# deemoe404/rmcv

Measured on AMD Instinct MI355X. Metric: frames/sec (1280x1024 BGR) armour detect, higher is better.
Workload: dtype u8

## Files before the change

### rmcv_amd/csrc/k_contours.hip

```cpp
#include "contours_device.h"

namespace rmcv {

#define KC_KERNEL k_contours_w8
#define KC_THREADS 512
#include "k_contours_kernel.inc"
#undef KC_KERNEL
#undef KC_THREADS

static_assert(sizeof(ContoursLds) >= (CT_THREADS_MAX / 64) * sizeof(WaveLds), "the fit rows reuse the contour tables");

bool sparse_lean_applies(const Geom& g, const Bufs& b)
{
    return g.sparse_lean && !g.dense_defer && g.contour_tier == 0 && b.mid && g.h <= CT_MAXH && g.ww <= 32;
}

static hipError_t launch_contours_x(const Geom& g, const Bufs& b, const Limits& lim, const SparseTail& X, int waves, hipStream_t s)
{
    SparseSched Q;
    Q.order = b.frame_order;
    const int grid = g.n_frames;
    static const int force_literal = getenv("RMCV_CONTOURS_LITERAL") ? atoi(getenv("RMCV_CONTOURS_LITERAL")) : 0;
    static bool attr_set[MAX_DEVICES] = {};
    if (!attr_set[g.device]) {
        hipError_t e = hipFuncSetAttribute(reinterpret_cast<const void*>(k_contours_w8), hipFuncAttributeMaxDynamicSharedMemorySize,
                                           (int)lds_bytes(CT_MAXH));
        if (e != hipSuccess) return e;
        attr_set[g.device] = true;
    }
    const int force = force_literal ? force_literal : g.contour_tier;
    if (waves == 4 && X.fused && !X.C.enabled && sparse_lean_applies(g, b) && force == 0) return launch_contours_lean(g, b, lim, X, 2, Q, grid, s);
    if (waves == 4) {
        const bool defer = g.dense_defer && (force & 3) == 0 && b.mid;
        if (g.dense_defer == 3 && !defer) return hipSuccess;
        hipError_t e = g.dense_defer == 3 ? hipSuccess : launch_contours_w4(g, b, lim, X, force | (defer ? 4 : 0), Q, grid, s);
        if (e != hipSuccess || !defer || g.dense_defer == 2) return e;
        const SparseSched& Q2 = Q;
        static const bool second_w4 = getenv("RMCV_DEFER_W4") && atoi(getenv("RMCV_DEFER_W4"));
        if (second_w4) return launch_contours_w4(g, b, lim, X, 2 | 8, Q2, grid, s);
        return launch(k_contours_w8, dim3(grid), dim3(512), lds_bytes(g.h), s, b.bits, b.rowmask, g.h, b.lab, b.neg, g.w,
                       g.h, g.ww, g.prow, g.plane_pitch, b.points, b.cont_start, b.cont_len, b.n_contours, b.n_points, b.status,
                       lim.max_contours, lim.max_points, 2 | 8, b.elig, b.n_elig, b.slot_kind, X, b.visit_xy, b.mid, b.mid_stride,
                       b.mid_slot_cap, Q2, lds_rows_cap(g.h));
    }
    return launch(k_contours_w8, dim3(grid), dim3(512), lds_bytes(g.h), s, b.bits, b.rowmask, g.h, b.lab, b.neg, g.w,
                       g.h, g.ww, g.prow, g.plane_pitch, b.points, b.cont_start, b.cont_len, b.n_contours, b.n_points, b.status,
                       lim.max_contours, lim.max_points, force, b.elig, b.n_elig, b.slot_kind, X, b.visit_xy, b.mid, b.mid_stride,
                       b.mid_slot_cap, Q, lds_rows_cap(g.h));
}

hipError_t launch_contours(const Geom& g, const Bufs& b, const Limits& lim, hipStream_t s)
{
    SparseTail X;
    memset(&X, 0, sizeof(X));
    return launch_contours_x(g, b, lim, X, 8, s);
}

hipError_t launch_sparse(const Geom& g, const Bufs& b, const Limits& lim, const rmcv_params& p, bool pairs, bool identity, int waves, hipStream_t s)
{
    SparseTail X;
    memset(&X, 0, sizeof(X));
    X.fused = 1;
    X.G = {p.tilt_max, p.ratio_lo, p.ratio_hi, p.area_lo, p.area_hi, g.overloads};
    X.slot_ell = b.slot_ell;
    FitTail& T = X.T;
    T.blobs = b.blobs;
    T.blob_src = b.blob_src;
    T.ellipses = b.ellipses;
    T.neg_idx = b.neg_idx;
    T.n_blobs = b.n_blobs;
    T.n_neg = b.n_neg;
    T.status = b.status;
    T.armours = b.armours;
    T.n_armours = b.n_armours;
    T.max_blobs = lim.max_blobs;
    T.max_armours = lim.max_armours;
    T.enemy = p.camp;
    T.do_pairs = pairs ? 1 : 0;
    T.angle_diff_max = p.angle_diff_max;
    T.shear_max = p.shear_max;
    T.length_ratio_max = p.length_ratio_max;
    T.ov = g.overloads;
    if (identity && pairs) X.C = classify_args(g, b);
    return launch_contours_x(g, b, lim, X, waves, s);
}

__device__ __forceinline__ void export_lists(const ExportArgs& a, int gtid, int nthreads)
{
    if (gtid < 12 && a.hdr_src[gtid]) a.hdr_dst[gtid] = *a.hdr_src[gtid];
    for (int k = 0; k < a.n_sec; k++) {
        const ExportSec& e = a.sec[k];
        int n = e.count ? e.count[0] + e.count_add : e.max_elems;
        n = n < 0 ? 0 : (n > e.max_elems ? e.max_elems : n);
        const int ndw = n * (e.elem_bytes >> 2);
        const uint32_t* src = static_cast<const uint32_t*>(e.src);
        uint32_t* dst = static_cast<uint32_t*>(e.dst);
        for (int i = gtid; i < ndw; i += nthreads) dst[i] = src[i];
    }
}

__global__ void k_export(ExportArgs a)
{
    export_lists(a, blockIdx.x * blockDim.x + threadIdx.x, gridDim.x * blockDim.x);
}

hipError_t launch_export(const ExportArgs& a, hipStream_t s)
{
    return launch(k_export, dim3(8), dim3(256), 0, s, a);
}

__global__ void k_pack_contours(const rmcv_point* __restrict__ points, const int32_t* __restrict__ cont_start,
                                const int32_t* __restrict__ cont_len, const int32_t* __restrict__ n_contours, int max_contours,
                                int max_points, rmcv_point* __restrict__ pts_out, int32_t* __restrict__ offs_out,
                                int32_t* __restrict__ hdr_out, const int32_t* __restrict__ status, ExportArgs ex)
// ... 95 lines not shown
```

### rmcv_amd/csrc/rmcv_host.hip

```cpp
#include <math.h>
#include <sched.h>
#include <time.h>
#include <stdio.h>
#include <stdlib.h>
#include <string.h>

#include <algorithm>
#include <vector>

#include "rmcv_internal.h"

using namespace rmcv;

struct rmcv_ctx {
    int device = 0;
    Limits lim{};
    Geom geom{};
    Bufs bufs{};
    hipStream_t stream = nullptr;
    hipEvent_t ev[6] = {};
    uint8_t* own_frames = nullptr;
    size_t own_frames_bytes = 0;
    rmcv_point* pack_pts = nullptr;
    int32_t* pack_offs = nullptr;
// ... 266 lines not shown
    if (e == hipSuccess) {
        hipDeviceProp_t prop;
        c->geom.device = device;
        c->geom.pixel_halo_nt = getenv("RMCV_K1_HALO_NT") ? atoi(getenv("RMCV_K1_HALO_NT")) : 0;
        c->geom.pixel_rowquad = getenv("RMCV_K1_LINEAR") && atoi(getenv("RMCV_K1_LINEAR")) == 0;
        if (getenv("RMCV_IMAGE_EXPORT")) c->image_export = atoi(getenv("RMCV_IMAGE_EXPORT"));
        if (getenv("RMCV_FRAME_UPLOAD")) c->frame_upload = atoi(getenv("RMCV_FRAME_UPLOAD"));
        c->geom.pixel_ws = 1;
        c->geom.dense_defer = getenv("RMCV_DENSE_DEFER") ? atoi(getenv("RMCV_DENSE_DEFER")) : 0;
        c->geom.n_cu = (device < MAX_DEVICES && hipGetDeviceProperties(&prop, device) == hipSuccess) ? prop.multiProcessorCount : 0;
        if (device >= MAX_DEVICES) e = hipErrorInvalidDevice;
    }
    const size_t F = (size_t)d.max_frames;
    const size_t plane = (size_t)(d.max_height + 2) * ((d.max_width + 63) / 64 + 2);
    Bufs& b = c->bufs;
    if (e == hipSuccess) e = dalloc(c, &b.binary, F * d.max_width * d.max_height);
    if (e == hipSuccess) e = dalloc(c, &b.bits, F * plane);
    if (e == hipSuccess) e = dalloc(c, &b.rowmask, F * d.max_height);
    if (e == hipSuccess) e = dalloc(c, &b.strip_ctr, 9 * CTR_STRIDE);
    if (e == hipSuccess) e = dalloc(c, &b.lab, F * plane);
    if (e == hipSuccess) e = dalloc(c, &b.neg, F * plane);
    if (e == hipSuccess) e = dalloc(c, &b.points, F * d.max_points);
    if (e == hipSuccess) e = dalloc(c, &c->pack_pts, F * d.max_points);
    if (e == hipSuccess) e = dalloc(c, &c->pack_offs, F * (d.max_contours + 1));
    if (e == hipSuccess) e = dalloc(c, &b.cont_start, F * d.max_contours);
    if (e == hipSuccess) e = dalloc(c, &b.cont_len, F * d.max_contours);
    if (e == hipSuccess) e = dalloc(c, &b.n_contours, F);
    if (e == hipSuccess) e = dalloc(c, &b.n_points, F);
    if (e == hipSuccess) e = dalloc(c, &b.visit_xy, F * VISIT_CAP);
    {
        const int64_t words = (int64_t)((d.max_width + 63) / 64) * d.max_height;
        b.mid_slot_cap = (int)std::min<int64_t>(words, 65535);
        b.mid_stride = (int64_t)((mid_bytes(b.mid_slot_cap) + 255) & ~(size_t)255);
        b.mid = nullptr;
    }
    if (e == hipSuccess) e = dalloc(c, &b.blobs, F * d.max_blobs);
    if (e == hipSuccess) e = dalloc(c, &b.blob_src, F * d.max_blobs);
    if (e == hipSuccess) e = dalloc(c, &b.ellipses, F * d.max_blobs);
    if (e == hipSuccess) e = dalloc(c, &b.neg_idx, F * d.max_contours);
    if (e == hipSuccess) e = dalloc(c, &b.elig, F * d.max_contours);
    if (e == hipSuccess) e = dalloc(c, &b.n_elig, F);
    if (e == hipSuccess) e = dalloc(c, &b.slot_kind, F * d.max_contours);
    if (e == hipSuccess) e = dalloc(c, &b.slot_ell, F * d.max_contours);
    if (e == hipSuccess) e = dalloc(c, &b.n_blobs, F);
    if (e == hipSuccess) e = dalloc(c, &b.n_neg, F);
    if (e == hipSuccess) e = dalloc(c, &b.armours, F * d.max_armours);
    if (e == hipSuccess) e = dalloc(c, &b.n_armours, F);
    if (e == hipSuccess) e = dalloc(c, &b.status, F);
    if (e == hipSuccess) e = dalloc(c, &b.frame_order, F);
    if (e == hipSuccess) e = dalloc(c, &c->order_scratch, 2 * F);
    if (e == hipSuccess) {
        hipMemset(b.strip_ctr, 0, 9 * CTR_STRIDE * sizeof(int));
        hipMemset(b.n_contours, 0, F * 4);
        hipMemset(b.n_points, 0, F * 4);
        hipMemset(b.n_blobs, 0, F * 4);
        hipMemset(b.n_neg, 0, F * 4);
        hipMemset(b.n_armours, 0, F * 4);
        e = hipMemset(b.status, 0, F * 4);
    }
    if (e != hipSuccess) {
        fprintf(stderr, "rmcv_ctx_create: %s\n", hipGetErrorString(e));
        rmcv_ctx_destroy(c);
        return e == hipErrorOutOfMemory ? RMCV_ERR_NOMEM : RMCV_ERR_HIP;
    }
    *out = c;
    return RMCV_OK;
}

}

namespace rmcv {
void ctx_external_order(rmcv_ctx* c, hipEvent_t done)
{
    c->external_order = true;
    c->ext_done = done;
}
const Limits& ctx_limits(const rmcv_ctx* c) { return c->lim; }
void ctx_pixel_shape(rmcv_ctx* c, int shape) { c->geom.pixel_ws = shape ? 1 : 0; }
uint64_t ctx_blocking_calls(const rmcv_ctx* c) { return c->blocking_calls; }
int ctx_wait_timeout_ms(const rmcv_ctx* c) { return c->wait_timeout_ms; }
bool pixel_ws_full(const rmcv_ctx* c, int lower_bound) { return binary_ws_full(c->geom, c->bufs, lower_bound); }
void ctx_defer_phase(rmcv_ctx* c, int phase) { c->geom.dense_defer = phase; }
void ctx_sparse_lean(rmcv_ctx* c, int on) { c->geom.sparse_lean = on ? 1 : 0; }
int ctx_input_format(const rmcv_ctx* c) { return c->input_format; }
int ctx_compact(rmcv_ctx* c, void* d_armours_out, int cap, void* d_frame_offs, void* d_status_or, hipStream_t s, void* hd_record, int host_head)
{
    HIPCHK(c, launch_compact_armours(c->geom, c->bufs, c->lim, (rmcv_armour*)d_armours_out, cap, (int32_t*)d_frame_offs, s, (int32_t*)d_status_or, (uint8_t*)hd_record, host_head), "k_compact_armours");
    return RMCV_OK;
}
}

static void resident_none(rmcv_ctx* c)
{
    c->res_nc = c->res_nb = -1;
    c->ahead_lb = c->ahead_ar = false;
}

static int ensure_own_frames(rmcv_ctx* c, size_t need)
{
    if (need <= c->own_frames_bytes) return RMCV_OK;
    if (c->own_frames) hipFree(c->own_frames);
    c->own_frames = nullptr;
    c->own_frames_bytes = 0;
    size_t cap = (size_t)((3 * c->lim.max_width + 15) & ~15) * c->lim.max_height * c->lim.max_frames;
    if (cap < need) cap = need;
    HIPCHK(c, hipMalloc((void**)&c->own_frames, cap), "hipMalloc frames");
    c->own_frames_bytes = cap;
    return RMCV_OK;
}

static int ensure_staging(rmcv_ctx* c)
{
    if (c->h_hdr) return RMCV_OK;
    const Limits& L = c->lim;
    hipError_t e = hipHostMalloc((void**)&c->h_hdr, 16 * sizeof(int32_t), hipHostMallocDefault);
    if (e == hipSuccess) e = hipHostMalloc((void**)&c->h_pts, (size_t)L.max_points * sizeof(rmcv_point), hipHostMallocDefault);
    if (e == hipSuccess) e = hipHostMalloc((void**)&c->h_offs, (size_t)(L.max_contours + 1) * 4, hipHostMallocDefault);
    if (e == hipSuccess) e = hipHostMalloc((void**)&c->h_blobs, (size_t)L.max_blobs * sizeof(rmcv_lightblob), hipHostMallocDefault);
    if (e == hipSuccess) e = hipHostMalloc((void**)&c->h_blob_src, (size_t)L.max_blobs * 4, hipHostMallocDefault);
    if (e == hipSuccess) e = hipHostMalloc((void**)&c->h_neg, (size_t)L.max_contours * 4, hipHostMallocDefault);
    if (e == hipSuccess) e = hipHostMalloc((void**)&c->h_armours, (size_t)L.max_armours * sizeof(rmcv_armour), hipHostMallocDefault);
    if (e == hipSuccess) e = dalloc(c, &c->d_hdr, 16);
    if (e != hipSuccess) return fail(c, RMCV_ERR_NOMEM, "pinned staging", e);
    memset(c->h_hdr, 0, 16 * sizeof(int32_t));
    if (hipHostGetDevicePointer((void**)&c->hd_hdr, c->h_hdr, 0) != hipSuccess || hipHostGetDevicePointer((void**)&c->hd_pts, c->h_pts, 0) != hipSuccess ||
        hipHostGetDevicePointer((void**)&c->hd_offs, c->h_offs, 0) != hipSuccess || hipHostGetDevicePointer((void**)&c->hd_blobs, c->h_blobs, 0) != hipSuccess ||
        hipHostGetDevicePointer((void**)&c->hd_blob_src, c->h_blob_src, 0) != hipSuccess || hipHostGetDevicePointer((void**)&c->hd_neg, c->h_neg, 0) != hipSuccess ||
        hipHostGetDevicePointer((void**)&c->hd_armours, c->h_armours, 0) != hipSuccess) {
        (void)hipGetLastError();
        c->hd_hdr = nullptr;
    }
    return RMCV_OK;
}

static int ensure_mid(rmcv_ctx* c, int n_frames)
{
    if (n_frames <= c->mid_frames || c->mid_failed) return RMCV_OK;
    const bool no_mid = getenv("RMCV_NO_MID") && atoi(getenv("RMCV_NO_MID"));
    c->blocking_calls++;
    if (c->bufs.mid) {
        const int rcs = rmcv_batch_sync(c);
        if (rcs) return rcs;
        uint8_t* raw = c->bufs.mid - GUARD;
        for (size_t i = 0; i < c->allocs.size(); i++)
            if (c->allocs[i] == raw) { c->allocs.erase(c->allocs.begin() + i); break; }
        for (size_t i = 0; i < c->guarded.size(); i++)
            if (c->guarded[i].base == raw) { c->guarded.erase(c->guarded.begin() + i); break; }
        (void)hipFree(raw);
        c->bufs.mid = nullptr;
        c->mid_frames = 0;
    }
    const int want = n_frames > 1 ? c->lim.max_frames : 1;
    uint8_t* m = nullptr;
    const hipError_t e = no_mid ? hipErrorOutOfMemory : dalloc_named(c, &m, (size_t)want * (size_t)c->bufs.mid_stride, "b.mid");
    if (e != hipSuccess) {
        (void)hipGetLastError();
        c->mid_failed = true;
        return RMCV_OK;
    }
    c->bufs.mid = m;
    c->mid_frames = want;
    return RMCV_OK;
}

namespace rmcv {
static constexpr int ORDER_LDS = 2048;
// ... 1408 lines not shown
```

### rmcv_amd/csrc/rmcv_internal.h

```cpp
#pragma once
#include <hip/hip_runtime.h>
#include <stdint.h>

#include <tuple>
#include <utility>

#include "../../include/rmcv_abi.h"

namespace rmcv {

struct Geom {
    int device;
    int n_cu;
    int pixel_halo_nt;
    int pixel_rowquad;
    int pixel_ws;
    int dense_defer;
    int overloads;
    int sparse_lean;
    int contour_tier;
    int input_format;
    int n_frames;
    int w, h;
    int stride;
    int64_t frame_pitch;
    int ww;
    int prow;
    int64_t plane_pitch;
};

static constexpr int CTR_STRIDE = 32;
#ifndef RMCV_SR
#define RMCV_SR 32
#endif
static constexpr int STRIP_ROWS = RMCV_SR;
static constexpr int VISIT_CAP = 4096;
static constexpr int NN_MID = 1 << 17;
static constexpr int CAND_MID = 1 << 15;
inline size_t mid_bytes(int slot_cap)
{
    return (size_t)slot_cap * (6 * 8 + 2 * 4) + (size_t)NN_MID * (2 * 8 + 2 * 4) + (size_t)CAND_MID * 4 * 4;
}

struct Limits {
    int max_frames, max_width, max_height, max_contours, max_points, max_blobs, max_armours;
};

struct Bufs {
    const uint8_t* frames;
    uint8_t* binary;
    uint64_t* bits;
    int* strip_ctr;
    uint32_t* rowmask;
    uint64_t* lab;
    uint64_t* neg;
    rmcv_point* points;
    int32_t* cont_start;
    int32_t* cont_len;
    int32_t* n_contours;
    int32_t* n_points;
    uint32_t* visit_xy;
    uint8_t* mid;
    int64_t mid_stride;
    int mid_slot_cap;
    rmcv_lightblob* blobs;
    int32_t* blob_src;
    rmcv_rrect* ellipses;
    int32_t* elig;
    int32_t* n_elig;
    int32_t* slot_kind;
    rmcv_rrect* slot_ell;
    int32_t* neg_idx;
    int32_t* n_blobs;
    int32_t* n_neg;
    rmcv_armour* armours;
    int32_t* n_armours;
    int32_t* status;
    int32_t* frame_order;
    float* svm_w;
    double* svm_rho;
    int32_t* svm_labels;
    int svm_classes;
    int32_t* identity;
    uint8_t* icons;
    rmcv_pnp_config* pnp_cfg;
    double* base2gripper;
    double* poses;
};

#define RMCV_FRAME_DEFERRED_ (1 << 30)

struct SparseSched {
    const int32_t* order;
};

static constexpr int MAX_DEVICES = 64;

template <typename... P, size_t... I>
inline hipError_t launch_tuple(void (*kernel)(P...), dim3 grid, dim3 block, size_t lds, hipStream_t s, std::tuple<P...>& vals,
                               std::index_sequence<I...>)
{
    void* ptrs[] = {static_cast<void*>(const_cast<typename std::remove_const<P>::type*>(&std::get<I>(vals)))...};
    return hipLaunchKernel(reinterpret_cast<const void*>(kernel), grid, block, ptrs, lds, s);
}
template <typename... P, typename... A>
inline hipError_t launch(void (*kernel)(P...), dim3 grid, dim3 block, size_t lds, hipStream_t s, A&&... a)
{
    static_assert(sizeof...(P) == sizeof...(A), "argument count differs from the kernel's parameter list");
    std::tuple<P...> vals{static_cast<P>(a)...};
    return launch_tuple(kernel, grid, block, lds, s, vals, std::index_sequence_for<P...>{});
}

int64_t pixel_ws_launches();
hipError_t launch_match(const Geom& g, const Bufs& b, const Limits& lim, const rmcv_params& p, const rmcv_legacy_params& lp,
                        int mode, bool with_frames, bool pairs, hipStream_t s);
hipError_t launch_sparse(const Geom& g, const Bufs& b, const Limits& lim, const rmcv_params& p, bool pairs, bool identity, int waves, hipStream_t s);
hipError_t launch_pnp(const Geom& g, const Bufs& b, const Limits& lim, hipStream_t s);
hipError_t launch_binary(const Geom& g, const Bufs& b, int camp, int lower_bound, int morph, bool image, int groups, hipStream_t s);
bool binary_ws_full(const Geom& g, const Bufs& b, int lower_bound);
hipError_t launch_binary_bayer(const Geom& g, const Bufs& b, int camp, int lower_bound, int morph, bool image, hipStream_t s);
hipError_t launch_demosaic(const uint8_t* d_raw, int stride, int w, int h, int pattern, uint8_t* d_out, int out_stride, hipStream_t s);
bool sparse_lean_applies(const Geom& g, const Bufs& b);
hipError_t launch_contours(const Geom& g, const Bufs& b, const Limits& lim, hipStream_t s);
hipError_t launch_blobs(const Geom& g, const Bufs& b, const Limits& lim, const rmcv_params& p, hipStream_t s);
hipError_t launch_armours(const Geom& g, const Bufs& b, const Limits& lim, const rmcv_params& p, hipStream_t s);
hipError_t launch_blobs_armours(const Geom& g, const Bufs& b, const Limits& lim, const rmcv_params& p, hipStream_t s);
hipError_t launch_compact_armours(const Geom& g, const Bufs& b, const Limits& lim, rmcv_armour* d_out, int cap,
                                  int32_t* d_frame_offs, hipStream_t s, int32_t* d_status_or = nullptr, uint8_t* hd_record = nullptr, int host_head = 0);
hipError_t launch_status_clear(const Geom& g, const Bufs& b, int mask, hipStream_t s);
hipError_t launch_classify(const Geom& g, const Bufs& b, const Limits& lim, hipStream_t s);
hipError_t launch_pack_bits(const Geom& g, const Bufs& b, hipStream_t s);
struct ExportSec {
    const void* src;
    void* dst;
    const int32_t* count;
    int count_add, elem_bytes, max_elems;
};
struct ExportArgs {
    ExportSec sec[8];
    int n_sec;
    const int32_t* hdr_src[12];
    int32_t* hdr_dst;
};
hipError_t launch_export(const ExportArgs& a, hipStream_t s);
hipError_t launch_pack_contours(const Geom& g, const Bufs& b, const Limits& lim, rmcv_point* d_pts_out, int32_t* d_offs_out,
                                int32_t* d_hdr , hipStream_t s, const ExportArgs* ex = nullptr);
hipError_t launch_gather3(const int32_t* a, const int32_t* b, const int32_t* c, int32_t* d_out, hipStream_t s);

void ctx_external_order(rmcv_ctx* c, hipEvent_t done);
int ctx_compact(rmcv_ctx* c, void* d_armours_out, int cap, void* d_frame_offs, void* d_status_or, hipStream_t s, void* hd_record = nullptr, int host_head = 0);
const Limits& ctx_limits(const rmcv_ctx* c);
void ctx_pixel_shape(rmcv_ctx* c, int shape);
int ctx_bind_frames(rmcv_ctx* c, const void* d_frames, int n_frames, int w, int h, int stride, int64_t frame_pitch, hipStream_t s);
int ctx_prepare_ring(rmcv_ctx* c);
uint64_t ctx_blocking_calls(const rmcv_ctx* c);
int ctx_wait_timeout_ms(const rmcv_ctx* c);
bool pixel_ws_full(const rmcv_ctx* c, int lower_bound);
int wait_stream_deadline(hipStream_t s, int timeout_ms, hipError_t* err);
int wait_event_deadline(hipEvent_t ev, int timeout_ms, hipError_t* err);
hipError_t launch_delay(unsigned long long ns, hipStream_t s);
int ctx_check_stages(rmcv_ctx* c, const rmcv_params* p, int stages);
void ctx_defer_phase(rmcv_ctx* c, int phase);
void ctx_sparse_lean(rmcv_ctx* c, int on);
int ctx_input_format(const rmcv_ctx* c);

}
```

### rmcv_amd/csrc/rmcv_pipeline.hip

```cpp
#include <stdio.h>
#include <stdlib.h>
#include <string.h>
#include <time.h>

#include <new>
#include <vector>

#include "rmcv_internal.h"

using namespace rmcv;


struct rmcv_pipeline {
    int device = 0;
    rmcv_pipeline_config cfg{};
    Limits lim{};
    int64_t head_bytes = 0, record_bytes = 0;
    std::vector<rmcv_ctx*> ring;
    std::vector<hipStream_t> pix, sp, dn;
    std::vector<hipEvent_t> ev_bin, ev_done, ev_host, ev_sp;
    std::vector<void*> ev_hook;
    std::vector<uint8_t*> d_rec, h_rec, hd_rec;
    std::vector<uint64_t> slot_ticket;
    std::vector<int> slot_frames;
    std::vector<hipStream_t> slot_stream;
    uint64_t next_ticket = 0, collected = 0;
    int hot = 0;
    bool calm = false;
    uint64_t hot_seq = 0, hot_batches = 0;
    std::vector<int> ctx_last;
    std::vector<int> slot_ctx;
    std::vector<hipEvent_t> ev_free;
    struct Pending {
        bool valid = false;
        uint64_t t = 0;
        size_t k = 0;
        rmcv_ctx* c = nullptr;
        rmcv_params p{};
        rmcv_legacy_params lp{};
        bool has_lp = false, used = false, heavy = false;
        int sparse = 0, n_frames = 0;
        hipStream_t B = nullptr;
    } pend;
    uint64_t latency_batches = 0;
    bool lazy_back = true;
    bool chain_cold = true, was_cold = false;
    int chain_cold_us = 60;
    bool early_free = true;
    bool heavy = false;
    int heavy_pixel_groups = 0;
    uint64_t heavy_batches = 0;
    std::vector<char> slot_lean;
    bool split_now = false;
    uint64_t split_batches = 0;
    rmcv_pipeline_hook hook = nullptr;
    void* hook_user = nullptr;
    rmcv_comm* comm = nullptr;
    int root = 0, n_ranks = 0, rank = 0;
    std::vector<uint8_t*> d_recv;
    hipEvent_t ev_gather = nullptr;
    bool gather_pending = false;
    uint64_t blocking_base = 0, own_blocking = 0, held_back = 0;
    std::vector<hipEvent_t> ev_chg;
    int wait_timeout_ms = 5000;
    const char* last_what = "nothing";
    int hot_cfg = 0;
    int64_t hot_plane_bytes = 0;
    bool ws_always = false;
    bool hot_identity = false;
    double max_submit_us = 0;
    char err[256] = {0};
};

static int finish_back(rmcv_pipeline* pl, bool latency);
static int hot_for(const rmcv_pipeline* pl, int n_frames, int w, int h);

static int pfail(rmcv_pipeline* pl, int code, const char* what, hipError_t e = hipSuccess)
{
    if (pl) {
        if (e != hipSuccess) snprintf(pl->err, sizeof(pl->err), "%s: %s", what, hipGetErrorString(e));
        else snprintf(pl->err, sizeof(pl->err), "%s", what);
    }
    if (e != hipSuccess) (void)hipGetLastError();
    return code;
}
#define PCHK(pl, call, what)                                               \
    do {                                                                   \
        (pl)->last_what = what;                                            \
        hipError_t e__ = (call);                                           \
        if (e__ != hipSuccess) return pfail((pl), RMCV_ERR_HIP, what, e__); \
    } while (0)
static int cfail(rmcv_pipeline* pl, rmcv_ctx* c, int rc)
{
    snprintf(pl->err, sizeof(pl->err), "%s", rmcv_last_error(c));
    return rc;
}

static int pwait_event(rmcv_pipeline* pl, hipEvent_t ev, const char* what)
{
    hipError_t e = hipSuccess;
    const int rcw = wait_event_deadline(ev, pl->wait_timeout_ms, &e);
    if (rcw < 0) return pfail(pl, RMCV_ERR_HIP, what, e);
    if (rcw > 0) {
        snprintf(pl->err, sizeof(pl->err), "%s: not finished after %d ms (rmcv_pipeline_set_wait_timeout); enqueued last: %s", what, pl->wait_timeout_ms, pl->last_what);
        return RMCV_ERR_TIMEOUT;
    }
    return RMCV_OK;
}
static int pwait_stream(rmcv_pipeline* pl, hipStream_t st, const char* what)
{
    hipError_t e = hipSuccess;
    const int rcw = wait_stream_deadline(st, pl->wait_timeout_ms, &e);
    if (rcw < 0) return pfail(pl, RMCV_ERR_HIP, what, e);
    if (rcw > 0) {
        snprintf(pl->err, sizeof(pl->err), "%s: not finished after %d ms (rmcv_pipeline_set_wait_timeout); enqueued last: %s", what, pl->wait_timeout_ms, pl->last_what);
        return RMCV_ERR_TIMEOUT;
    }
    return RMCV_OK;
}
static uint64_t ring_blocking(const rmcv_pipeline* pl)
{
    uint64_t n = 0;
    for (auto c : pl->ring) n += ctx_blocking_calls(c);
    return n;
}

extern "C" {

void rmcv_default_pipeline_config(rmcv_pipeline_config* c)
{
    if (!c) return;
    memset(c, 0, sizeof(*c));
    c->depth = 8;
    c->pixel_streams = 2;
    c->sparse_streams = 4;
    c->armour_cap = 0;
    c->sparse_waves = 4;
    c->pixel_groups = 2;
    c->host_results = 1;
    c->dense_streams = 4;
    c->hot_contexts = 0;
}

void rmcv_pipeline_destroy(rmcv_pipeline* pl)
{
    if (!pl) return;
    hipSetDevice(pl->device);
    if (!pl->ring.empty()) (void)finish_back(pl, true);
    {
        bool stuck = false;
        for (auto s : pl->pix) if (s) stuck |= pwait_stream(pl, s, "destroy") == RMCV_ERR_TIMEOUT;
// ... 56 lines not shown
    for (int k = 0; k < d.depth && rc == RMCV_OK; k++) {
        rmcv_ctx* c = nullptr;
        rc = rmcv_ctx_create(device, limits, &c);
        if (rc == RMCV_OK) {
            pl->ring.push_back(c);
            rc = rmcv_ctx_set_option(c, RMCV_OPT_SPARSE_WAVES, d.sparse_waves);
            if (rc == RMCV_OK) rc = rmcv_ctx_set_option(c, RMCV_OPT_PIXEL_GROUPS, d.pixel_groups);
            if (rc == RMCV_OK) rc = ctx_prepare_ring(c);
        }
    }
    if (rc != RMCV_OK) {
        rmcv_pipeline_destroy(pl);
        return rc;
    }
    pl->lim = ctx_limits(pl->ring[0]);
    if (pl->cfg.armour_cap <= 0) pl->cfg.armour_cap = 8 * pl->lim.max_frames;
    pl->head_bytes = (((int64_t)pl->lim.max_frames + 3) * 4 + 15) / 16 * 16;
    pl->record_bytes = pl->head_bytes + (int64_t)pl->cfg.armour_cap * (int64_t)sizeof(rmcv_armour);
    hipError_t e = hipSetDevice(device);
    int lo = 0, hi = 0;
    if (e == hipSuccess) e = hipDeviceGetStreamPriorityRange(&lo, &hi);
    for (int i = 0; i < d.pixel_streams && e == hipSuccess; i++) {
        hipStream_t s = nullptr;
        e = hipStreamCreateWithPriority(&s, hipStreamNonBlocking, 0);
        pl->pix.push_back(s);
    }
    for (int i = 0; i < d.sparse_streams && e == hipSuccess; i++) {
        hipStream_t s = nullptr;
        e = hipStreamCreateWithPriority(&s, hipStreamNonBlocking, hi);
        pl->sp.push_back(s);
    }
    const unsigned dev_flags = hipEventDisableTiming;
    for (int i = 0; i < d.dense_streams && e == hipSuccess; i++) {
        hipStream_t s = nullptr;
        e = hipStreamCreateWithPriority(&s, hipStreamNonBlocking, 0);
        pl->dn.push_back(s);
    }
    for (int k = 0; k < d.depth && e == hipSuccess; k++) {
        hipEvent_t a = nullptr, b = nullptr, h = nullptr, sp_ = nullptr;
        if (e == hipSuccess) e = hipEventCreateWithFlags(&sp_, hipEventDisableTiming);
        pl->ev_sp.push_back(sp_);
        hipEvent_t fr_ = nullptr, chg_ = nullptr;
        if (e == hipSuccess) e = hipEventCreateWithFlags(&fr_, hipEventDisableTiming);
        pl->ev_free.push_back(fr_);
        if (e == hipSuccess) e = hipEventCreateWithFlags(&chg_, hipEventDisableTiming);
        pl->ev_chg.push_back(chg_);
        uint8_t *dr = nullptr, *hr = nullptr;
        e = hipEventCreateWithFlags(&a, dev_flags);
        if (e == hipSuccess) e = hipEventCreateWithFlags(&b, dev_flags);
        if (e == hipSuccess) e = hipEventCreateWithFlags(&h, hipEventDisableTiming);
        if (e == hipSuccess) e = hipMalloc((void**)&dr, (size_t)pl->record_bytes);
        if (e == hipSuccess) e = hipMemset(dr, 0, (size_t)pl->record_bytes);
        uint8_t* hdr = nullptr;
        if (e == hipSuccess && d.host_results == 1) {
            e = hipHostMalloc((void**)&hr, (size_t)pl->record_bytes, hipHostMallocMapped);
            if (e == hipSuccess) memset(hr, 0, (size_t)pl->record_bytes);
            if (e == hipSuccess) e = hipHostGetDevicePointer((void**)&hdr, hr, 0);
        }
        pl->hd_rec.push_back(hdr);
        pl->ev_bin.push_back(a);
        pl->ev_done.push_back(b);
        pl->ev_host.push_back(h);
        pl->d_rec.push_back(dr);
        pl->h_rec.push_back(hr);
        pl->ev_hook.push_back(nullptr);
        pl->slot_ticket.push_back(0);
        pl->slot_frames.push_back(0);
        pl->slot_stream.push_back(nullptr);
        if (e == hipSuccess) ctx_external_order(pl->ring[(size_t)k], b);
    }
    if (e == hipSuccess) e = hipEventCreateWithFlags(&pl->ev_gather, hipEventDisableTiming);
    pl->ctx_last.assign((size_t)d.depth, -1);
    pl->slot_lean.assign((size_t)d.depth, 0);
    pl->slot_ctx.assign((size_t)d.depth, 0);
    pl->hot = hot_for(pl, pl->lim.max_frames, pl->lim.max_width, pl->lim.max_height);
    pl->wait_timeout_ms = ctx_wait_timeout_ms(pl->ring[0]);
#ifdef RMCV_DEV_KNOBS
    pl->lazy_back = !(getenv("RMCV_LAZY_BACK") && atoi(getenv("RMCV_LAZY_BACK")) == 0);
    pl->chain_cold = !(getenv("RMCV_CHAIN_COLD") && atoi(getenv("RMCV_CHAIN_COLD")) == 0);
    if (getenv("RMCV_CHAIN_COLD")) pl->chain_cold_us = atoi(getenv("RMCV_CHAIN_COLD")) > 1 ? atoi(getenv("RMCV_CHAIN_COLD")) : 0;
    pl->early_free = !(getenv("RMCV_EARLY_FREE") && atoi(getenv("RMCV_EARLY_FREE")) == 0);
    if (getenv("RMCV_HOT_IDENTITY")) pl->hot_identity = atoi(getenv("RMCV_HOT_IDENTITY")) != 0;
    if (getenv("RMCV_WS_ALWAYS")) pl->ws_always = atoi(getenv("RMCV_WS_ALWAYS")) != 0;
    if (getenv("RMCV_HEAVY_PG")) pl->heavy_pixel_groups = atoi(getenv("RMCV_HEAVY_PG")) > 0 ? atoi(getenv("RMCV_HEAVY_PG")) : 0;
    if (getenv("RMCV_HEAVY_OFF") && atoi(getenv("RMCV_HEAVY_OFF"))) pl->heavy_pixel_groups = -1;
#endif
    pl->blocking_base = ring_blocking(pl);
    if (e != hipSuccess) {
        fprintf(stderr, "rmcv_pipeline_create: %s\n", hipGetErrorString(e));
        (void)hipGetLastError();
        rmcv_pipeline_destroy(pl);
        return e == hipErrorOutOfMemory ? RMCV_ERR_NOMEM : RMCV_ERR_HIP;
    }
    *out = pl;
    return RMCV_OK;
}

int rmcv_hw_queues_hint(void)
{
    setenv("GPU_MAX_HW_QUEUES", "12", 0);
    const char* q = getenv("GPU_MAX_HW_QUEUES");
    return q ? atoi(q) : 0;
}

const char* rmcv_pipeline_last_error(const rmcv_pipeline* pl) { return pl ? pl->err : "null pipeline"; }

int rmcv_pipeline_get_info(const rmcv_pipeline* pl, rmcv_pipeline_info* o)
{
    if (!pl || !o) return RMCV_ERR_BAD_ARG;
    memset(o, 0, sizeof(*o));
    o->depth = pl->cfg.depth;
    o->pixel_streams = pl->cfg.pixel_streams;
    o->sparse_streams = pl->cfg.sparse_streams;
    o->armour_cap = pl->cfg.armour_cap;
    o->sparse_waves = pl->cfg.sparse_waves;
    o->pixel_groups = pl->cfg.pixel_groups;
    o->host_results = pl->cfg.host_results;
    o->dense_streams = pl->cfg.dense_streams;
    o->max_frames = pl->lim.max_frames;
    const char* q = getenv("GPU_MAX_HW_QUEUES");
    o->hw_queues_env = q ? atoi(q) : 0;
    o->hw_queues_wanted = 1 + pl->cfg.pixel_streams + pl->cfg.sparse_streams + pl->cfg.dense_streams + (pl->comm ? 1 : 0);
    o->record_bytes = pl->record_bytes;
    o->armours_offset = pl->head_bytes;
    o->submitted = pl->next_ticket;
    o->collected = pl->collected;
    o->dense_split = pl->split_batches;
    o->hot_batches = pl->hot_batches;
    o->hot_contexts = pl->hot;
    o->latency_batches = pl->latency_batches;
    o->host_blocking_calls = pl->own_blocking;
    o->max_submit_us = pl->max_submit_us;
    o->wait_timeout_ms = pl->wait_timeout_ms;
    o->held_back = pl->held_back;
    o->heavy_batches = pl->heavy_batches;
    return RMCV_OK;
}

rmcv_ctx* rmcv_pipeline_context(rmcv_pipeline* pl, int slot)
{
    if (!pl || slot < 0 || slot >= pl->cfg.depth) return nullptr;
    return pl->ring[(size_t)slot];
}

int rmcv_pipeline_set_hot_contexts(rmcv_pipeline* pl, int n)
{
    if (!pl) return RMCV_ERR_BAD_ARG;
    if (n <= 0) { pl->hot = 0; pl->hot_cfg = -1; return RMCV_OK; }
    if (n < 3 || n >= pl->cfg.depth) return pfail(pl, RMCV_ERR_BAD_ARG, "hot_contexts: 3 .. depth - 1, or 0 / -1 for off");
    if (pl->cfg.host_results != 1 || pl->cfg.sparse_waves != 4) return pfail(pl, RMCV_ERR_BAD_ARG, "hot_contexts needs host_results = 1 and sparse_waves = 4");
    pl->hot = pl->hot_cfg = n;
    return RMCV_OK;
}

int rmcv_pipeline_set_wait_timeout(rmcv_pipeline* pl, int ms)
{
    if (!pl || ms < 0) return RMCV_ERR_BAD_ARG;
    pl->wait_timeout_ms = ms;
    for (auto c : pl->ring) rmcv_ctx_set_option(c, RMCV_OPT_WAIT_TIMEOUT_MS, ms);
    return RMCV_OK;
}

static int hot_for(const rmcv_pipeline* pl, int n_frames, int w, int h)
{
    if (pl->hot_cfg != 0) return pl->hot_cfg > 0 ? pl->hot_cfg : 0;
    const int64_t plane = (int64_t)n_frames * (h + 2) * ((w + 63) / 64 + 2) * 8;
// ... 97 lines not shown
                rc = rmcv_batch_run(c, p, sparse, T);
            }
            ctx_defer_phase(c, 0);
        } else {
            if (heavy) ctx_sparse_lean(c, 1);
            rc = lp ? rmcv_batch_run_legacy(c, p, lp, sparse, B) : rmcv_batch_run(c, p, sparse, B);
            if (heavy) ctx_sparse_lean(c, 0);
        }
        if (rc) return cfail(pl, c, rc);
    }
    PCHK(pl, hipEventRecord(pl->ev_free[k], T), "pipeline: mark the pixel outputs' last reader");
    if (pl->ev_hook[k]) {
        PCHK(pl, hipStreamWaitEvent(T, (hipEvent_t)pl->ev_hook[k], 0), "pipeline: wait for the record's reader");
        pl->ev_hook[k] = nullptr;
    }
    int32_t* offs = reinterpret_cast<int32_t*>(pl->d_rec[k]);
    rc = ctx_compact(c, pl->d_rec[k] + pl->head_bytes, pl->cfg.armour_cap, offs, offs + pl->lim.max_frames + 1, T, pl->hd_rec[k], (int)pl->head_bytes);
    if (rc) return cfail(pl, c, rc);
    PCHK(pl, hipEventRecord(pl->ev_done[k], T), "pipeline: mark the slot");
    pl->slot_ticket[k] = t + 1;
    pl->slot_frames[k] = n_frames;
    pl->slot_lean[k] = heavy ? 1 : 0;
    pl->slot_stream[k] = T;
    if (pl->comm) {
        if (pl->gather_pending) PCHK(pl, hipStreamWaitEvent(T, pl->ev_gather, 0), "pipeline: order the gathers");
        rc = rmcv_gather(pl->comm, pl->d_rec[k], pl->record_bytes, pl->rank == pl->root ? pl->d_recv[k] : nullptr, pl->root, T);
        if (rc) return pfail(pl, rc, rmcv_comm_last_error(pl->comm));
        PCHK(pl, hipEventRecord(pl->ev_gather, T), "pipeline: mark the gather");
        pl->gather_pending = true;
        PCHK(pl, hipEventRecord(pl->ev_host[k], T), "pipeline: mark the gather");
    } else if (pl->hook) {
        void* done = nullptr;
        rc = pl->hook(pl->hook_user, t, pl->d_rec[k], pl->record_bytes, T, &done);
        if (rc) return pfail(pl, rc, "the pipeline hook failed");
        pl->ev_hook[k] = done;
    }
    return RMCV_OK;
}

static int submit(rmcv_pipeline* pl, const void* d_frames, int n_frames, int w, int h, int stride, int64_t frame_pitch, const rmcv_params* p,
                  const rmcv_legacy_params* lp, int stages, uint64_t* ticket)
{
    if (!pl || !d_frames || !p) return RMCV_ERR_BAD_ARG;
    if (!(stages & RMCV_STAGE_BINARY)) return pfail(pl, RMCV_ERR_BAD_ARG, "a pipelined batch starts at RMCV_STAGE_BINARY");
    hipSetDevice(pl->device);
    { const int rcb = finish_back(pl, false); if (rcb) return rcb; }
    const uint64_t t = pl->next_ticket;
    const size_t k = (size_t)(t % (uint64_t)pl->cfg.depth);
    const bool used = pl->slot_ticket[k] != 0;
    pl->hot = hot_for(pl, n_frames, w, h);
    if (pl->cfg.host_results == 1) {
        for (uint64_t d = 1; d <= (uint64_t)pl->cfg.depth && d <= t; d++) {
            const size_t s_ = (size_t)((t - d) % (uint64_t)pl->cfg.depth);
            if (pl->slot_ticket[s_] != t - d + 1 || !pl->h_rec[s_]) break;
            if (hipEventQuery(pl->ev_done[s_]) != hipSuccess) continue;
            const uint32_t word2 = reinterpret_cast<const uint32_t*>(pl->h_rec[s_])[pl->lim.max_frames + 2];
            const int dense = (int)(word2 & 0xFFFFFu), points = (int)(word2 >> 20) * 16;
            pl->heavy = pl->slot_lean[s_] ? points >= 1200 : (dense * 8 > pl->slot_frames[s_] || points >= 1500);
            pl->calm = dense == 0 && !pl->heavy;
            break;
        }
        (void)hipGetLastError();
    }
    const bool heavy = pl->heavy && pl->heavy_pixel_groups >= 0 && pl->cfg.host_results == 1 && pl->cfg.sparse_waves == 4 && pl->cfg.dense_streams >= 0 && !lp &&
                       !(stages & (RMCV_STAGE_IDENTITY | RMCV_STAGE_POSE)) && (stages & RMCV_STAGE_CONTOURS) && (stages & RMCV_STAGE_BLOBS);
    const bool fast = pl->hot && pl->calm && !lp && !(stages & RMCV_STAGE_POSE) && (pl->hot_identity || !(stages & RMCV_STAGE_IDENTITY));
    const size_t j = fast ? (size_t)(pl->hot_seq % (uint64_t)pl->hot) : k;
    rmcv_ctx* c = pl->ring[j];
    if (lp && ctx_input_format(c)) return pfail(pl, RMCV_ERR_BAD_ARG, "the legacy matcher votes camps from BGR means: not for Bayer frames (RMCV_OPT_INPUT_FORMAT)");
    hipStream_t A = pl->pix[(size_t)(t % (uint64_t)pl->cfg.pixel_streams)], B = pl->sp[k % (size_t)pl->cfg.sparse_streams];
    int rc;
    if (used) PCHK(pl, hipStreamWaitEvent(A, pl->ev_done[k], 0), "pipeline: wait for the slot");
    if (pl->ctx_last[j] >= 0 && pl->ctx_last[j] != (int)k) {
        const size_t last = (size_t)pl->ctx_last[j];
        const bool early = pl->early_free && pl->slot_stream[last] == B;
        PCHK(pl, hipStreamWaitEvent(A, early ? pl->ev_free[last] : pl->ev_done[last], 0), "pipeline: wait for the context");
    }
    rc = ctx_bind_frames(c, d_frames, n_frames, w, h, stride, frame_pitch, A);
    if (rc) return cfail(pl, c, rc);
    if ((rc = ctx_check_stages(c, p, stages))) return cfail(pl, c, rc);
    const int pixel = stages & (RMCV_STAGE_BINARY | RMCV_STAGE_NO_IMAGE), sparse = stages & ~(RMCV_STAGE_BINARY | RMCV_STAGE_NO_IMAGE);
    ctx_external_order(c, pl->ev_done[k]);
    ctx_pixel_shape(c, (fast || pl->ws_always) ? 1 : 0);
    bool cold = false;
    if (fast && pl->chain_cold) {
        cold = t == 0;
        const size_t s_ = t ? (size_t)((t - 1) % (uint64_t)pl->cfg.depth) : 0;
        if (t > 0) {
            cold = pl->slot_ticket[s_] == t && hipEventQuery(pl->ev_done[s_]) == hipSuccess;
            (void)hipGetLastError();
        }
        if (!cold && pl->was_cold && pl->slot_ticket[s_] == t && pixel_ws_full(c, p->lower_bound)) {
            const double launch_us = (double)n_frames * 4.0 * w * h / 5.5e6;
            const int hold_us = launch_us < 100.0 ? 0 : (int)(launch_us / 4.0 < pl->chain_cold_us ? launch_us / 4.0 : pl->chain_cold_us);
            if (pl->chain_cold_us > 0) {
                if (hold_us > 0) {
                    PCHK(pl, launch_delay((unsigned long long)hold_us * 1000ull, A), "pipeline: k_delay");
                    pl->held_back++;
                }
            } else
                PCHK(pl, hipStreamWaitEvent(A, pl->ev_bin[s_], 0), "pipeline: chain a burst's second launch");
        }
    }
    if (heavy && pl->heavy_pixel_groups > 0) rmcv_ctx_set_option(c, RMCV_OPT_PIXEL_GROUPS, pl->heavy_pixel_groups);
    rc = rmcv_batch_run(c, p, pixel, A);
    if (heavy && pl->heavy_pixel_groups > 0) rmcv_ctx_set_option(c, RMCV_OPT_PIXEL_GROUPS, pl->cfg.pixel_groups);
    if (rc) return cfail(pl, c, rc);
    pl->last_what = ctx_input_format(c) ? "the pixel kernel (k_binary_bayer)" : "the pixel kernel (k_binary / k_binary_ws)";
    pl->was_cold = cold;
    if (fast) { pl->hot_seq++; pl->hot_batches++; }
    if (heavy) pl->heavy_batches++;
    pl->ctx_last[j] = (int)k;
    pl->slot_ctx[k] = (int)j;
    PCHK(pl, hipEventRecord(pl->ev_bin[k], A), "pipeline: mark the pixel kernel");
    PCHK(pl, hipStreamWaitEvent(B, pl->ev_bin[k], 0), "pipeline: chain the sparse stages");
    pl->next_ticket = t + 1;
    if (ticket) *ticket = t;
    pl->pend.valid = true;
    pl->pend.t = t;
    pl->pend.k = k;
    pl->pend.c = c;
    pl->pend.p = *p;
    pl->pend.has_lp = lp != nullptr;
    if (lp) pl->pend.lp = *lp;
    pl->pend.used = used;
    pl->pend.heavy = heavy;
    pl->pend.sparse = sparse;
    pl->pend.n_frames = n_frames;
    pl->pend.B = B;
    if (!pl->lazy_back || pl->hook || pl->comm) return finish_back(pl, false);
    return RMCV_OK;
}

static int submit_counted(rmcv_pipeline* pl, const void* d_frames, int n_frames, int w, int h, int stride, int64_t frame_pitch, const rmcv_params* p,
                          const rmcv_legacy_params* lp, int stages, uint64_t* ticket)
{
    if (!pl) return RMCV_ERR_BAD_ARG;
    timespec t0, t1;
    clock_gettime(CLOCK_MONOTONIC, &t0);
    const uint64_t b0 = ring_blocking(pl);
    const int rc = submit(pl, d_frames, n_frames, w, h, stride, frame_pitch, p, lp, stages, ticket);
    pl->own_blocking += ring_blocking(pl) - b0;
    clock_gettime(CLOCK_MONOTONIC, &t1);
    const double us = (t1.tv_sec - t0.tv_sec) * 1e6 + (t1.tv_nsec - t0.tv_nsec) * 1e-3;
    if (us > pl->max_submit_us) pl->max_submit_us = us;
    return rc;
}

int rmcv_pipeline_reset_stats(rmcv_pipeline* pl)
{
    if (!pl) return RMCV_ERR_BAD_ARG;
    pl->max_submit_us = 0;
    return RMCV_OK;
}

int rmcv_pipeline_submit(rmcv_pipeline* pl, const void* d_frames, int n_frames, int w, int h, int stride, int64_t frame_pitch,
                         const rmcv_params* p, int stages, uint64_t* ticket)
{
    return submit_counted(pl, d_frames, n_frames, w, h, stride, frame_pitch, p, nullptr, stages, ticket);
}

int rmcv_pipeline_submit_legacy(rmcv_pipeline* pl, const void* d_frames, int n_frames, int w, int h, int stride, int64_t frame_pitch,
                                const rmcv_params* p, const rmcv_legacy_params* lp, int stages, uint64_t* ticket)
{
    if (!lp) return RMCV_ERR_BAD_ARG;
    return submit_counted(pl, d_frames, n_frames, w, h, stride, frame_pitch, p, lp, stages, ticket);
// ... 128 lines not shown
```

### rmcv_amd/csrc/wave_detect.h

```cpp
#pragma once
#include "device_classify.h"
#include "device_fit.h"
#include "rmcv_internal.h"

namespace rmcv {

__device__ __forceinline__ int lanes_below(uint64_t m, int lane) { return __popcll(m & ((1ull << lane) - 1)); }

struct WaveLds {
    double rows[64][6];
    double terms[64];
    double dm[32];
};

__device__ __forceinline__ double wave_sum_f64(double v)
{
    for (int d = 32; d >= 1; d >>= 1) v += __shfl_xor(v, d);
    return v;
}
__device__ __forceinline__ long long wave_sum_i64(long long v)
{
    for (int d = 32; d >= 1; d >>= 1) v += __shfl_xor(v, d);
    return v;
}
// ... 453 lines not shown
        if (lane == 0) atomicOr(&status[f], RMCV_FRAME_OVF_BLOBS);
        np = max_blobs;
    }
    if (lane == 0) {
        n_blobs[f] = np;
        n_neg[f] = nn;
    }
    return np;
}

__device__ __forceinline__ bool pair_ok(const rmcv_lightblob& a, const rmcv_lightblob& b, float angle_diff_max,
                                        float shear_max, float length_ratio_max, int ov)
{
    const float angle_difference = abs_ov(a.angle - b.angle, ov);
    if (angle_difference > angle_diff_max) return false;
    const float y = abs_ov(a.center[1] - b.center[1], ov);
    const float x = abs_ov(a.center[0] - b.center[0], ov);
    const float rect_angle = atan2_deg_ov(y, x, ov);
    const float shear_i = abs_ov(a.angle > 90 ? abs_ov(a.angle - rect_angle, ov) - 90 : abs_ov(180 - a.angle - rect_angle, ov) - 90, ov);
    const float shear_j = abs_ov(b.angle > 90 ? abs_ov(b.angle - rect_angle, ov) - 90 : abs_ov(180 - b.angle - rect_angle, ov) - 90, ov);
    if (shear_i > shear_max || shear_j > shear_max) return false;
    const float hi = a.size[1], hj = b.size[1];
    const float mn = hi < hj ? hi : hj, mx = hi < hj ? hj : hi;
    if (mn / mx < length_ratio_max) return false;
    if (abs_ov(a.center[1] - b.center[1], ov) > (a.size[1] + b.size[1]) / 2) return false;
    if (abs_ov(a.center[0] - b.center[0], ov) > (a.size[1] + b.size[1]) * 2) return false;
    return true;
}

__device__ inline void armours_frame(int f, int lane, const rmcv_lightblob* blobs, int n, int max_blobs, float angle_diff_max,
                                     float shear_max, float length_ratio_max, int enemy, rmcv_armour* armours, int32_t* n_armours,
                                     int32_t* status, int max_armours, int ov)
{
    const rmcv_lightblob* lb = blobs + (int64_t)f * max_blobs;
    rmcv_armour* out = armours + (int64_t)f * max_armours;
    int na = 0;
    if (n >= 2) {
        const int total = n * (n - 1) / 2;
        int i = 0, rem = lane;
        while (i < n - 1 && rem >= n - 1 - i) { rem -= n - 1 - i; i++; }
        for (int base = 0; base < total; base += 64) {
            const int j = i + 1 + rem;
            bool ok = false;
            rmcv_lightblob a, b;
            if (base + lane < total) {
                a = lb[i];
                b = lb[j];
                ok = a.target == enemy && b.target == enemy && pair_ok(a, b, angle_diff_max, shear_max, length_ratio_max, ov);
            }
            const uint64_t m = __ballot(ok);
            if (ok) {
                const int o = na + lanes_below(m, lane);
                if (o < max_armours) {
                    make_armour(&a, &b, &out[o], ov);
                    out[o].blob_i = i;
                    out[o].blob_j = j;
                }
            }
            na += __popcll(m);
            rem += 64;
            while (i < n - 1 && rem >= n - 1 - i) { rem -= n - 1 - i; i++; }
        }
    }
    if (lane == 0) {
        if (na > max_armours) {
            atomicOr(&status[f], RMCV_FRAME_OVF_ARMOURS);
            na = max_armours;
        }
        n_armours[f] = na;
    }
}

struct SparseTail {
    int fused;
    FitGates G;
    rmcv_rrect* slot_ell;
    FitTail T;
    ClassifyArgs C;
};

hipError_t launch_contours_w4(const Geom& g, const Bufs& b, const Limits& lim, const SparseTail& X, int force_literal, const SparseSched& Q, int grid,
                              hipStream_t s);
hipError_t launch_contours_lean(const Geom& g, const Bufs& b, const Limits& lim, const SparseTail& X, int flags, const SparseSched& Q, int grid, hipStream_t s);

}
```

Baseline: 1.114 million.

## Add a lean 256-thread contours kernel for the calm hot path

Adds a new contours kernel variant compiled with smaller caps (slot, kept and neighbour tables), 256 threads, a VGPR limit and classification compiled out. It is selected in the pipeline's fast (hot and calm) path when the lean and defer modes are off. The goal is to let two contour workgroups share a CU with the binary kernel, cutting LDS and register pressure and raising overlap. The risk is that the reduced caps overflow on busier frames and that the register cap causes spills.

Result: no change. 1.124 million (median of 6 runs) (+1.0%).

```diff
diff --git a/rmcv_amd/csrc/k_contours.hip b/rmcv_amd/csrc/k_contours.hip
--- a/rmcv_amd/csrc/k_contours.hip
+++ b/rmcv_amd/csrc/k_contours.hip
@@ -30,6 +30,7 @@
     }
     const int force = force_literal ? force_literal : g.contour_tier;
     if (waves == 4 && X.fused && !X.C.enabled && sparse_lean_applies(g, b) && force == 0) return launch_contours_lean(g, b, lim, X, 2, Q, grid, s);
+    if (waves == 4 && X.fused && !X.C.enabled && g.sparse_calm && !g.sparse_lean && !g.dense_defer && force == 0) return launch_contours_calm(g, b, lim, X, Q, grid, s);
     if (waves == 4) {
         const bool defer = g.dense_defer && (force & 3) == 0 && b.mid;
         if (g.dense_defer == 3 && !defer) return hipSuccess;
diff --git a/rmcv_amd/csrc/k_contours_calm.hip b/rmcv_amd/csrc/k_contours_calm.hip
--- /dev/null
+++ b/rmcv_amd/csrc/k_contours_calm.hip
@@ -0,0 +1,39 @@
+#define RMCV_SLOT_CAP 1280
+#define RMCV_KEPT_CAP 128
+#define RMCV_NN_CAP 3072
+#define RMCV_CT_THREADS_MAX 256
+#ifndef RMCV_CALM_NUM_VGPR
+#define RMCV_CALM_NUM_VGPR 56
+#endif
+#define RMCV_KC_ATTR __attribute__((amdgpu_num_vgpr(RMCV_CALM_NUM_VGPR)))
+#include "contours_device.h"
+
+#include <algorithm>
+
+namespace rmcv {
+
+#define KC_KERNEL k_contours_calm
+#define KC_THREADS 256
+#define KC_NO_CLASSIFY
+#include "k_contours_kernel.inc"
+#undef KC_NO_CLASSIFY
+#undef KC_KERNEL
+#undef KC_THREADS
+
+static_assert(sizeof(ContoursLds) + (size_t)1024 * 8 <= 68 * 1024, "two of these workgroups (1280x1024) and k_binary_ws share a CU's 160 KB");
+
+hipError_t launch_contours_calm(const Geom& g, const Bufs& b, const Limits& lim, const SparseTail& X, const SparseSched& Q, int grid, hipStream_t s)
+{
+    static bool attr_set[MAX_DEVICES] = {};
+    if (!attr_set[g.device]) {
+        hipError_t e = hipFuncSetAttribute(reinterpret_cast<const void*>(k_contours_calm), hipFuncAttributeMaxDynamicSharedMemorySize, (int)lds_bytes(CT_MAXH));
+        if (e != hipSuccess) return e;
+        attr_set[g.device] = true;
+    }
+    return launch(k_contours_calm, dim3(grid), dim3(256), lds_bytes(g.h), s, b.bits, b.rowmask, g.h, b.lab, b.neg, g.w,
+                  g.h, g.ww, g.prow, g.plane_pitch, b.points, b.cont_start, b.cont_len, b.n_contours, b.n_points, b.status,
+                  lim.max_contours, lim.max_points, 0, b.elig, b.n_elig, b.slot_kind, X, b.visit_xy, b.mid, b.mid_stride,
+                  b.mid_slot_cap, Q, lds_rows_cap(g.h));
+}
+
+}
diff --git a/rmcv_amd/csrc/rmcv_host.hip b/rmcv_amd/csrc/rmcv_host.hip
--- a/rmcv_amd/csrc/rmcv_host.hip
+++ b/rmcv_amd/csrc/rmcv_host.hip
@@ -372,6 +372,7 @@
 bool pixel_ws_full(const rmcv_ctx* c, int lower_bound) { return binary_ws_full(c->geom, c->bufs, lower_bound); }
 void ctx_defer_phase(rmcv_ctx* c, int phase) { c->geom.dense_defer = phase; }
 void ctx_sparse_lean(rmcv_ctx* c, int on) { c->geom.sparse_lean = on ? 1 : 0; }
+void ctx_sparse_calm(rmcv_ctx* c, int on) { c->geom.sparse_calm = on ? 1 : 0; }
 int ctx_input_format(const rmcv_ctx* c) { return c->input_format; }
 int ctx_compact(rmcv_ctx* c, void* d_armours_out, int cap, void* d_frame_offs, void* d_status_or, hipStream_t s, void* hd_record, int host_head)
 {
diff --git a/rmcv_amd/csrc/rmcv_internal.h b/rmcv_amd/csrc/rmcv_internal.h
--- a/rmcv_amd/csrc/rmcv_internal.h
+++ b/rmcv_amd/csrc/rmcv_internal.h
@@ -18,6 +18,7 @@
     int dense_defer;
     int overloads;
     int sparse_lean;
+    int sparse_calm;
     int contour_tier;
     int input_format;
     int n_frames;
@@ -162,6 +163,7 @@
 int ctx_check_stages(rmcv_ctx* c, const rmcv_params* p, int stages);
 void ctx_defer_phase(rmcv_ctx* c, int phase);
 void ctx_sparse_lean(rmcv_ctx* c, int on);
+void ctx_sparse_calm(rmcv_ctx* c, int on);
 int ctx_input_format(const rmcv_ctx* c);
 
 }
diff --git a/rmcv_amd/csrc/rmcv_pipeline.hip b/rmcv_amd/csrc/rmcv_pipeline.hip
--- a/rmcv_amd/csrc/rmcv_pipeline.hip
+++ b/rmcv_amd/csrc/rmcv_pipeline.hip
@@ -67,6 +67,7 @@
     int hot_cfg = 0;
     int64_t hot_plane_bytes = 0;
     bool ws_always = false;
+    bool calm_kernel = true;
     bool hot_identity = false;
     double max_submit_us = 0;
     char err[256] = {0};
@@ -289,6 +290,7 @@
     pl->early_free = !(getenv("RMCV_EARLY_FREE") && atoi(getenv("RMCV_EARLY_FREE")) == 0);
     if (getenv("RMCV_HOT_IDENTITY")) pl->hot_identity = atoi(getenv("RMCV_HOT_IDENTITY")) != 0;
     if (getenv("RMCV_WS_ALWAYS")) pl->ws_always = atoi(getenv("RMCV_WS_ALWAYS")) != 0;
+    if (getenv("RMCV_CALM_KERNEL")) pl->calm_kernel = atoi(getenv("RMCV_CALM_KERNEL")) != 0;
     if (getenv("RMCV_HEAVY_PG")) pl->heavy_pixel_groups = atoi(getenv("RMCV_HEAVY_PG")) > 0 ? atoi(getenv("RMCV_HEAVY_PG")) : 0;
     if (getenv("RMCV_HEAVY_OFF") && atoi(getenv("RMCV_HEAVY_OFF"))) pl->heavy_pixel_groups = -1;
 #endif
@@ -552,6 +554,7 @@
     const int pixel = stages & (RMCV_STAGE_BINARY | RMCV_STAGE_NO_IMAGE), sparse = stages & ~(RMCV_STAGE_BINARY | RMCV_STAGE_NO_IMAGE);
     ctx_external_order(c, pl->ev_done[k]);
     ctx_pixel_shape(c, (fast || pl->ws_always) ? 1 : 0);
+    ctx_sparse_calm(c, (fast && pl->calm_kernel) ? 1 : 0);
     bool cold = false;
     if (fast && pl->chain_cold) {
         cold = t == 0;
diff --git a/rmcv_amd/csrc/wave_detect.h b/rmcv_amd/csrc/wave_detect.h
--- a/rmcv_amd/csrc/wave_detect.h
+++ b/rmcv_amd/csrc/wave_detect.h
@@ -559,5 +559,6 @@
 hipError_t launch_contours_w4(const Geom& g, const Bufs& b, const Limits& lim, const SparseTail& X, int force_literal, const SparseSched& Q, int grid,
                               hipStream_t s);
 hipError_t launch_contours_lean(const Geom& g, const Bufs& b, const Limits& lim, const SparseTail& X, int flags, const SparseSched& Q, int grid, hipStream_t s);
-
-}
+hipError_t launch_contours_calm(const Geom& g, const Bufs& b, const Limits& lim, const SparseTail& X, const SparseSched& Q, int grid, hipStream_t s);
+
+}
```
